# kawshik8/GAN-Image-Captioning

Hardware: AMD Instinct MI355X
Metric: captions/sec (G+D train step) (higher is better)
Workload: dtype bf16; 1 GPU; cfg2: adversarial G+D step, batch 64/GPU, 224x224 images, caption len 20, V=10000, E=H=512, 1-layer LSTM G, CNN-seq D (R=64,F=900), ResNet-50-shaped encoder, --conditional-gan 1; global_batch=64, caption_len=20, image_size=224, vocab=10000, conditional_gan=1, encoder=resnet50, step_impl=fused, parallelism=dp1

## Files before the change

gan-image-captioning_amd/csrc/gemm.h:

```cpp
#pragma once
#include "common.h"

namespace gic {

enum GemmEpi { EPI_PLAIN = 0, EPI_HIGHWAY = 1, EPI_BNSTATS = 2, EPI_GUMBELMAX = 3 };

struct GemmDesc {
  const void* A = nullptr;
  const void* B = nullptr;
  void* C = nullptr;
  int M = 0, N = 0, K = 0;
  long lda = 0, ldb = 0, ldc = 0;
  int a_kc = 1, b_kc = 1;
  int in_dtype = DT_F32, out_dtype = DT_F32;
  const float* bias = nullptr;
  int accumulate = 0;
  int c_zeroed = 0;
  int no_split = 0;
  float alpha = 1.f;
  int epi = EPI_PLAIN;
  const void* X = nullptr; long ldx = 0;
  union { float* Hpre = nullptr; float* a_sum2; };
  union { long ldh = 0; long ldc2; };
  const uint8_t* mask = nullptr; long ldmask = 0;
  uint8_t* mask_out = nullptr; long ldmask_out = 0;
  float keep_scale = 1.f;
  union { int use_philox = 0; int wgrad; }; float drop_p = 0.f; uint64_t seed = 0, stream = 0;
  const uint64_t* seed_dev = nullptr;
  int conv = 0;
  int cH = 0, cW = 0, cCin = 0, cHo = 0, cWo = 0, cKH = 0, cKW = 0, cStride = 1, cPad = 0;
  union { float* stats = nullptr; float* a_sum; };
  int stats_nrep = 1;
  const float* in_stats = nullptr; int in_nrep = 1;
  const float* in_gamma = nullptr; const float* in_beta = nullptr;
  float in_inv_count = 0.f;
  const void* res = nullptr;
  const float* res_stats = nullptr; int res_nrep = 1;
  const float* res_gamma = nullptr; const float* res_beta = nullptr;
  float res_inv_count = 0.f;
  union { void* out_wb = nullptr; void* C2; };
  unsigned long long* gm_rowkey = nullptr;
  const float* gm_bias = nullptr;
  const float* gm_u = nullptr; long gm_ldu = 0;
  float gm_temperature = 1.f;
  int n_fast = 0;
  union { int stats_only = 0; int n_split; };
  int dbg = 0;
};

int gemm(const GemmDesc& d, hipStream_t stream);


struct ConvBase {
  const void* A; const void* B; void* C; float* stats;
  const float* in_stats; const float* in_gamma; const float* in_beta;
  int M, N, lda, ldb, ldc, stats_nrep, in_nrep;
  float in_inv_count;
  unsigned a_bytes, b_bytes;
};

inline bool bn_in_args_ok(const GemmDesc& d) { return d.in_gamma && d.in_beta && d.in_inv_count > 0.f; }

bool conv_base(const GemmDesc& d, long a_elems, long b_elems, ConvBase& b);

bool wgrad_folds_a_sum(const GemmDesc& d);
int wgrad_tile_n(const GemmDesc& d);
void wgrad_launch_counts(long* launches, long* two_matrix);

bool route_only();
char* route_line();
constexpr int kRouteLen = 160;

int gemm_gumbelmax(const GemmDesc& d, hipStream_t stream);
long gemm_gumbelmax_from_cols(int in_dtype, int M, int K, long lda, long ldb);

}
```

gan-image-captioning_amd/csrc/gemm.hip:

```cpp
#include "gemm.h"
#include "conv3x3.h"
#include "conv1x1_stream.h"
#include "conv1x1_panel.h"
#include "conv1x1_pix.h"
#include "conv_stem.h"
#include "bn_fold.h"
#include "gemm_device.h"
#include "kernels.h"

#include <stdlib.h>
#include <string.h>
#include <atomic>

namespace gic {

namespace {

typedef __attribute__((address_space(3))) bf16x4 lds_bf16x4;
typedef const __attribute__((address_space(1))) u32x4* gptr_u4;

__device__ __attribute__((aligned(16))) unsigned int g_zero16[4] = {0u, 0u, 0u, 0u};
typedef const __attribute__((address_space(1))) void* gbl_void_ptr;

#ifdef GIC_STAMPS
}
__device__ unsigned long long g_stamp[32];
namespace {
#define STAMP(i) do { if (tid == 0 && blockIdx.y == 0 && (blockIdx.x == 0 || blockIdx.x == gridDim.x - 1)) { \
  const int o_ = blockIdx.x == 0 ? 0 : 16; g_stamp[o_ + 2 * (i)] = __builtin_amdgcn_s_memtime(); g_stamp[o_ + 2 * (i) + 1] = __builtin_amdgcn_s_memrealtime(); } } while (0)
#define DBG d.dbg
#else
#define STAMP(i) do {} while (0)
#define DBG 0
#endif

template <typename T> struct GlobalPtr { typedef const __attribute__((address_space(1))) T* type; };

template <typename TI, bool KC, int BR, int S, int NC>
__device__ __forceinline__ void g4_store(unsigned char* img, const u32x4 (&reg)[NC], const int tid) {
#pragma unroll
  for (int i = 0; i < NC; ++i) {
    const int c = tid + i * 256;
    if constexpr (KC) {
      *(u32x4*)(img + (c >> 3) * S + (c & 7) * 16) = reg[i];
    } else {
      constexpr int CPR = BR / (16 / (int)sizeof(TI));
      *(u32x4*)(img + (c / CPR) * S + (c % CPR) * 16) = reg[i];
    }
  }
}
template <typename TI, bool KC, int BR, int S>
__device__ __forceinline__ void g4_store_scalar(unsigned char* img, const typename GlobalPtr<TI>::type P, const long ld, const int row0,
                                                const int R, const int k0, const int K, const int tid) {
  constexpr int SZ = sizeof(TI), BK = 128 / SZ;
  for (int e = tid; e < BR * BK; e += 256) {
    TI v = (TI)0.f;
    if constexpr (KC) {
      const int row = e / BK, kk = e % BK;
      const int r = row0 + row, k = k0 + kk;
      if (r < R && k < K) v = P[(long)r * ld + k];
      *(TI*)(img + row * S + kk * SZ) = v;
    } else {
      const int kk = e / BR, row = e % BR;
      const int r = row0 + row, k = k0 + kk;
      if (r < R && k < K) v = P[(long)k * ld + r];
      *(TI*)(img + kk * S + row * SZ) = v;
    }
  }
}
template <bool KC, bool PIPE, int S>
__device__ __forceinline__ bf16x8 g4_frag_bf16(const unsigned char* img, const int r0, const int ks, const int lr, const int lg) {
  if constexpr (PIPE) {
    return *(const bf16x8*)(img + (r0 + lr) * 128 + swz_chunk(r0 + lr, ks * 4 + lg));
  } else if constexpr (KC) {
    return *(const bf16x8*)(img + (r0 + lr) * S + ks * 64 + lg * 16);
  } else {
    const unsigned char* p0 = img + (ks * 32 + lg * 8 + (lr >> 2)) * S + (r0 + 4 * (lr & 3)) * 2;
    const bf16x4 t0 = __builtin_amdgcn_ds_read_tr16_b64_v4bf16((lds_bf16x4*)p0);
    const bf16x4 t1 = __builtin_amdgcn_ds_read_tr16_b64_v4bf16((lds_bf16x4*)(p0 + 4 * S));
    return __builtin_shufflevector(t0, t1, 0, 1, 2, 3, 4, 5, 6, 7);
  }
}
template <bool KC, bool PIPE, int S>
__device__ __forceinline__ void g4_frag_f32(float (&f)[8], const unsigned char* img, const int r0, const int lr, const int lg) {
  if constexpr (KC) {
    const int row = r0 + lr;
    const float4 v0 = *(const float4*)(img + row * S + (PIPE ? swz_chunk(row, 2 * lg) : 2 * lg * 16));
    const float4 v1 = *(const float4*)(img + row * S + (PIPE ? swz_chunk(row, 2 * lg + 1) : (2 * lg + 1) * 16));
    f[0] = v0.x; f[1] = v0.y; f[2] = v0.z; f[3] = v0.w;
    f[4] = v1.x; f[5] = v1.y; f[6] = v1.z; f[7] = v1.w;
  } else {
#pragma unroll
    for (int s = 0; s < 8; ++s) f[s] = *(const float*)(img + (lg * 8 + s) * S + (r0 + lr) * 4);
  }
}

std::atomic<long> g_wgrad_launches{0}, g_wgrad_two{0};

constexpr int EPI_WGRAD = 4;

__device__ __forceinline__ void g4_chunk_add(float (&s)[8], const u32x4 r) {
  const bf16x8 v = __builtin_bit_cast(bf16x8, r);
#pragma unroll
  for (int e = 0; e < 8; ++e) s[e] += (float)v[e];
}

template <typename TI, typename TO, bool AKC, bool BKC, int BM, int BN, bool VEC, int EPI, bool CONV, bool PIPE>
__global__ __launch_bounds__(256) void gemm_kernel(const GemmDesc d, const int k_tiles_per_split) {
  static_assert(!CONV || (AKC && BKC && VEC), "the implicit-GEMM convolution loader is k-contiguous and vectorised");
  static_assert(!PIPE || (AKC && BKC && VEC), "the LDS-DMA pipeline needs k-contiguous 16-byte chunks");
  constexpr bool WG = EPI == EPI_WGRAD;
  static_assert(!WG || (!AKC && !BKC && VEC && !CONV && !PIPE && sizeof(TI) == 2), "the weight-gradient extras exist in the vectorised m/n-contiguous bf16 form only");
  constexpr int SZ = sizeof(TI);
  constexpr int BK = 128 / SZ;
  constexpr int VE = 16 / SZ;
  constexpr int SA = PIPE ? 128 : (AKC ? 144 : BM * SZ + 16);
  constexpr int SB = PIPE ? 128 : (BKC ? 144 : BN * SZ + 16);
  constexpr int NSTAGE = PIPE ? 3 : 2;
  constexpr int A_BYTES = AKC ? BM * SA : BK * SA;
  constexpr int B_BYTES = BKC ? BN * SB : BK * SB;
  constexpr int BUF_BYTES = A_BYTES + B_BYTES;
  constexpr int TM = BM / 32, TN = BN / 32;
  constexpr int CA = BM / 32, CB = BN / 32;
  constexpr bool IS_BF16 = (SZ == 2);
  typedef typename GlobalPtr<TI>::type gptr_t;

  constexpr int EPI_BYTES = BM * (BN * (int)sizeof(TO) + 16) + 4 * (BN / 2) * 2 * 4;
  constexpr int SMEM_BYTES = NSTAGE * BUF_BYTES > EPI_BYTES ? NSTAGE * BUF_BYTES : EPI_BYTES;
  __shared__ __attribute__((aligned(16))) unsigned char smem[SMEM_BYTES];

  const int tid = threadIdx.x, lane = tid & 63, w = tid >> 6;
  STAMP(0);
  const int wr = w >> 1, wc = w & 1;
  const int lr = lane & 15, lg = lane >> 4;

  const int tiles_m = (d.M + BM - 1) / BM;
  const int bid = xcd_run(blockIdx.x, gridDim.x);
  const int bm0 = (bid % tiles_m) * BM;
  const int bn0 = (bid / tiles_m) * BN;

  gptr_t A = (gptr_t)d.A;
  gptr_t B = (gptr_t)d.B;
  const int M = d.M, N = d.N, K = d.K;
  const long lda = d.lda, ldb = d.ldb;

  f32x4 acc[TM][TN];
#pragma unroll
  for (int i = 0; i < TM; ++i)
#pragma unroll
    for (int j = 0; j < TN; ++j) acc[i][j] = (f32x4){0.f, 0.f, 0.f, 0.f};

  u32x4 ra[CA], rb[CB];

  float asum[WG ? VE : 1];
  bool asum_on = false;
  if constexpr (WG) {
    asum_on = d.a_sum && bn0 == 0;
#pragma unroll
    for (int e = 0; e < VE; ++e) asum[e] = 0.f;
  }

  long cv_base[CONV ? CA : 1];
  int cv_hi0[CONV ? CA : 1], cv_wi0[CONV ? CA : 1];
  int cv_r = 0, cv_s = 0, cv_c = 0;
  if constexpr (CONV) {
#pragma unroll
    for (int i = 0; i < CA; ++i) {
      const int m = bm0 + ((tid + i * 256) >> 3);
      const ConvOrigin<long> o = conv_origin<long>(m, m < M, d.cHo, d.cWo, d.cH, d.cW, d.cStride, d.cPad);
      cv_hi0[i] = o.hi0; cv_wi0[i] = o.wi0; cv_base[i] = o.pix;
    }
    const int kchunk = PIPE ? swz_dma_chunk(tid) : (tid & 7);
    const int k = blockIdx.y * k_tiles_per_split * BK + kchunk * VE;
    cv_c = k % d.cCin;
    const int t = k / d.cCin;
    cv_s = t % d.cKW;
    cv_r = t / d.cKW;
  }

  auto gload = [&](int kt) {
    if constexpr (VEC) {
      const int k0 = kt * BK;
      if constexpr (CONV) {
#pragma unroll
        for (int i = 0; i < CA; ++i) {
          ra[i] = (u32x4){0u, 0u, 0u, 0u};
          const int hi = cv_hi0[i] + cv_r, wi = cv_wi0[i] + cv_s;
          if (cv_r < d.cKH && hi >= 0 && hi < d.cH && wi >= 0 && wi < d.cW)
            ra[i] = *(gptr_u4)(A + (cv_base[i] + (long)cv_r * d.cW + cv_s) * d.cCin + cv_c);
        }
      } else {
#pragma unroll
        for (int i = 0; i < CA; ++i) {
          const int c = tid + i * 256;
          ra[i] = (u32x4){0u, 0u, 0u, 0u};
          if constexpr (AKC) {
            const int m = bm0 + (c >> 3), k = k0 + (c & 7) * VE;
            if (m < M && k < K) ra[i] = *(gptr_u4)(A + (long)m * lda + k);
          } else {
            constexpr int CPR = BM / VE;
            const int k = k0 + c / CPR, m = bm0 + (c % CPR) * VE;
            if (k < K && m < M) ra[i] = *(gptr_u4)(A + (long)k * lda + m);
          }
        }
      }
#pragma unroll
      for (int i = 0; i < CB; ++i) {
        const int c = tid + i * 256;
        rb[i] = (u32x4){0u, 0u, 0u, 0u};
        if constexpr (BKC) {
          const int n = bn0 + (c >> 3), k = k0 + (c & 7) * VE;
          if (n < N && k < K) rb[i] = *(gptr_u4)(B + (long)n * ldb + k);
        } else {
          constexpr int CPR = BN / VE;
          const int k = k0 + c / CPR, n = bn0 + (c % CPR) * VE;
          if (k < K && n < N) rb[i] = *(gptr_u4)(B + (long)k * ldb + n);
        }
      }
      if constexpr (CONV) conv_tap_advance(cv_r, cv_s, cv_c, BK, d.cCin, d.cKW);
    }
  };

  auto sstore = [&](int kt, int buf) {
    unsigned char* sA = smem + buf * BUF_BYTES;
    unsigned char* sB = sA + A_BYTES;
    if constexpr (VEC) {
      if constexpr (WG) {
        if (asum_on) {
#pragma unroll
          for (int i = 0; i < CA; ++i) g4_chunk_add(asum, ra[i]);
        }
      }
      g4_store<TI, AKC, BM, SA>(sA, ra, tid);
      g4_store<TI, BKC, BN, SB>(sB, rb, tid);
    } else {
      g4_store_scalar<TI, AKC, BM, SA>(sA, A, lda, bm0, M, kt * BK, K, tid);
      g4_store_scalar<TI, BKC, BN, SB>(sB, B, ldb, bn0, N, kt * BK, K, tid);
    }
  };

  auto issue = [&](int kt, int buf) {
    if constexpr (PIPE) {
      unsigned char* sA = smem + buf * BUF_BYTES;
      unsigned char* sB = sA + A_BYTES;
      const int k0 = kt * BK;
      const int kc = swz_dma_chunk(tid) * VE;
      const int wbase = (tid & ~63) * 16;
#pragma unroll
      for (int i = 0; i < CA; ++i) {
        const int c = tid + i * 256;
        const TI* src = (const TI*)g_zero16;
        if constexpr (CONV) {
          const int hi = cv_hi0[i] + cv_r, wi = cv_wi0[i] + cv_s;
          if (cv_r < d.cKH && hi >= 0 && hi < d.cH && wi >= 0 && wi < d.cW)
            src = (const TI*)d.A + (cv_base[i] + (long)cv_r * d.cW + cv_s) * d.cCin + cv_c;
        } else {
          const int m = bm0 + (c >> 3), k = k0 + kc;
          if (m < M && k < K) src = (const TI*)d.A + (long)m * lda + k;
        }
        __builtin_amdgcn_global_load_lds((gbl_void_ptr)src, (lds_void_ptr)(sA + i * 4096 + wbase), 16, 0, 0);
      }
#pragma unroll
      for (int i = 0; i < CB; ++i) {
        const int c = tid + i * 256;
        const TI* src = (const TI*)g_zero16;
        const int n = bn0 + (c >> 3), k = k0 + kc;
        if (n < N && k < K) src = (const TI*)d.B + (long)n * ldb + k;
        __builtin_amdgcn_global_load_lds((gbl_void_ptr)src, (lds_void_ptr)(sB + i * 4096 + wbase), 16, 0, 0);
      }
      if constexpr (CONV) conv_tap_advance(cv_r, cv_s, cv_c, BK, d.cCin, d.cKW);
    }
  };

  auto compute = [&](int buf) {
    const unsigned char* sA = smem + buf * BUF_BYTES;
    const unsigned char* sB = sA + A_BYTES;
    if constexpr (IS_BF16) {
#pragma unroll
      for (int ks = 0; ks < BK / 32; ++ks) {
        bf16x8 fa[TM], fb[TN];
#pragma unroll
        for (int t = 0; t < TM; ++t) fa[t] = g4_frag_bf16<AKC, PIPE, SA>(sA, wr * (BM / 2) + t * 16, ks, lr, lg);
#pragma unroll
        for (int t = 0; t < TN; ++t) fb[t] = g4_frag_bf16<BKC, PIPE, SB>(sB, wc * (BN / 2) + t * 16, ks, lr, lg);
        mfma_block(acc, fa, fb);
      }
    } else {
      float fa[TM][8], fb[TN][8];
#pragma unroll
      for (int t = 0; t < TM; ++t) g4_frag_f32<AKC, PIPE, SA>(fa[t], sA, wr * (BM / 2) + t * 16, lr, lg);
#pragma unroll
      for (int t = 0; t < TN; ++t) g4_frag_f32<BKC, PIPE, SB>(fb[t], sB, wc * (BN / 2) + t * 16, lr, lg);
#pragma unroll
      for (int s = 0; s < 8; ++s)
#pragma unroll
        for (int i = 0; i < TM; ++i)
#pragma unroll
          for (int j = 0; j < TN; ++j)
            acc[i][j] = __builtin_amdgcn_mfma_f32_16x16x4f32(fa[i][s], fb[j][s], acc[i][j], 0, 0, 0);
    }
  };

  const int nk = (K + BK - 1) / BK;
  const int kt0 = blockIdx.y * k_tiles_per_split;
  const int kt1 = min(nk, kt0 + k_tiles_per_split);
  if constexpr (PIPE) {
    if (kt0 < kt1) {
      constexpr int NL = CA + CB;
      STAMP(1);
      issue(kt0, 0);
      if (kt0 + 1 < kt1) issue(kt0 + 1, 1);
      int buf = 0;
      for (int kt = kt0; kt < kt1; ++kt) {
        if (kt + 1 < kt1) asm volatile("s_waitcnt vmcnt(%0)" ::"n"(NL) : "memory");
        else asm volatile("s_waitcnt vmcnt(0)" ::: "memory");
        __builtin_amdgcn_s_barrier();
        if (kt == kt0) STAMP(2);
        if (kt + 2 < kt1 && !(DBG & 1)) issue(kt + 2, buf >= 1 ? buf - 1 : 2);
        if (!(DBG & 2)) compute(buf);
        buf = buf == 2 ? 0 : buf + 1;
      }
      __syncthreads();
      STAMP(3);
    }
  } else if (kt0 < kt1) {
    int cur = 0;
    gload(kt0);
    sstore(kt0, 0);
    __syncthreads();
    for (int kt = kt0; kt < kt1; ++kt) {
      const bool more = kt + 1 < kt1;
      if (more) gload(kt + 1);
      compute(cur);
      if (more) sstore(kt + 1, cur ^ 1);
      __syncthreads();
      cur ^= 1;
    }
  }

  TO* __restrict__ C = (TO*)d.C;
  long ldc = d.ldc;
#define LDC (WG ? ldc : d.ldc)
  const bool split = gridDim.y > 1;

  if constexpr (WG) {
    if (d.C2 && bn0 >= d.n_split) { C = (TO*)d.C2 - d.n_split; ldc = d.ldc2; }
    if (asum_on) {
      constexpr int CPR = BM / VE, G = 256 / CPR;
      static_assert(G * BM * 4 <= SMEM_BYTES, "the column-sum partials must fit the LDS allocation");
      float* sS = (float*)smem;
#pragma unroll
      for (int e = 0; e < VE; ++e) sS[(tid / CPR) * BM + (tid % CPR) * VE + e] = asum[e];
      __syncthreads();
      if (tid < BM && bm0 + tid < M) {
        float t = 0.f;
#pragma unroll
        for (int g = 0; g < G; ++g) t += sS[g * BM + tid];
        const int m = bm0 + tid;
        if (split) {
          atomicAdd(d.a_sum + m, t);
          if (d.a_sum2) atomicAdd(d.a_sum2 + m, t);
        } else {
          d.a_sum[m] = d.accumulate ? d.a_sum[m] + t : t;
          if (d.a_sum2) d.a_sum2[m] = d.accumulate ? d.a_sum2[m] + t : t;
        }
      }
      __syncthreads();
    }
  }

  if constexpr (EPI != EPI_HIGHWAY) {
    constexpr int OSZ = sizeof(TO);
    constexpr int OVE = 16 / OSZ;
    constexpr int SC = BN * OSZ + 16;
    static_assert(BM * SC + 4 * (BN / 2) * 2 * 4 <= SMEM_BYTES, "C tile + stats scratch must fit the LDS allocation");
    const bool staged = !split && !d.accumulate && (N % OVE == 0) && (LDC % OVE == 0) && ((((uintptr_t)(WG ? (const void*)C : (const void*)d.C)) & 15) == 0);
    if (staged) {
      unsigned char* sC = smem;
      float* sStat = (float*)(smem + BM * SC);
      float st_s[TN], st_q[TN];
#pragma unroll
      for (int j = 0; j < TN; ++j) {
        const int nl = wc * (BN / 2) + j * 16 + lr;
        const int n = bn0 + nl;
        const float bias = (d.bias && n < N) ? d.bias[n] : 0.f;
        st_s[j] = 0.f; st_q[j] = 0.f;
#pragma unroll
        for (int i = 0; i < TM; ++i) {
#pragma unroll
          for (int r = 0; r < 4; ++r) {
            const int ml = wr * (BM / 2) + i * 16 + lg * 4 + r;
            const float v = d.alpha * acc[i][j][r] + bias;
            *(TO*)(sC + ml * SC + nl * OSZ) = from_f32<TO>(v);
            if (EPI == EPI_BNSTATS && bm0 + ml < M) { st_s[j] += v; st_q[j] += v * v; }
          }
        }
        if constexpr (EPI == EPI_BNSTATS) {
          st_s[j] += __shfl_xor(st_s[j], 16, 64); st_q[j] += __shfl_xor(st_q[j], 16, 64);
          st_s[j] += __shfl_xor(st_s[j], 32, 64); st_q[j] += __shfl_xor(st_q[j], 32, 64);
          if (lg == 0) { sStat[(w * (BN / 2) + j * 16 + lr) * 2] = st_s[j]; sStat[(w * (BN / 2) + j * 16 + lr) * 2 + 1] = st_q[j]; }
        }
      }
      __syncthreads();
      STAMP(4);
      if constexpr (EPI == EPI_BNSTATS) {
        if (tid < BN) {
          const int cwc = tid / (BN / 2), cl = tid % (BN / 2), n = bn0 + tid;
          if (n < N) {
            const float s0 = sStat[((0 * 2 + cwc) * (BN / 2) + cl) * 2] + sStat[((1 * 2 + cwc) * (BN / 2) + cl) * 2];
            const float q0 = sStat[((0 * 2 + cwc) * (BN / 2) + cl) * 2 + 1] + sStat[((1 * 2 + cwc) * (BN / 2) + cl) * 2 + 1];
            float* st = d.stats + (long)(blockIdx.x % d.stats_nrep) * 2 * N;
            atomicAdd(&st[n], s0);
            atomicAdd(&st[N + n], q0);
          }
        }
      }
      constexpr int CPR = BN / OVE;
      for (int c = tid; c < BM * CPR; c += 256) {
        const int ml = c / CPR, cc = c % CPR;
        const int m = bm0 + ml, n = bn0 + cc * OVE;
        if (m < M && n < N) *(u32x4*)(C + (long)m * LDC + n) = *(const u32x4*)(sC + ml * SC + cc * 16);
      }
      STAMP(5);
      return;
    }
  }

#pragma unroll
  for (int i = 0; i < TM; ++i) {
#pragma unroll
    for (int j = 0; j < TN; ++j) {
      const int n = bn0 + wc * (BN / 2) + j * 16 + lr;
      if (n >= N) continue;
      const float bias = (d.bias && blockIdx.y == 0) ? d.bias[n] : 0.f;
      const int mb = bm0 + wr * (BM / 2) + i * 16 + lg * 4;
      float keep4[4] = {1.f, 1.f, 1.f, 1.f};
      if constexpr (EPI == EPI_HIGHWAY) {
        if (!d.mask && d.use_philox) highway_keep4(d.seed_dev ? *d.seed_dev : d.seed, d.stream, mb >> 2, N, n, d.drop_p, keep4);
      }
      float st_s = 0.f, st_q = 0.f;
#pragma unroll
      for (int r = 0; r < 4; ++r) {
        const int m = mb + r;
        if (m >= M) continue;
        float v = d.alpha * acc[i][j][r] + bias;
        if constexpr (EPI == EPI_BNSTATS) {
          C[(long)m * LDC + n] = from_f32<TO>(v);
          st_s += v; st_q += v * v;
        } else if constexpr (EPI == EPI_PLAIN || WG) {
          const long o = (long)m * LDC + n;
          if constexpr (sizeof(TO) == 4) {
            if (split) { atomicAdd((float*)&C[o], v); continue; }
          }
          if (d.accumulate) v += to_f32<TO>(C[o]);
          C[o] = from_f32<TO>(v);
        } else {
          const float y = highway_gate(v, to_f32<TI>(((const TI*)d.X)[(long)m * d.ldx + n]));
          if (d.Hpre) d.Hpre[(long)m * d.ldh + n] = v;
          float keep = keep4[r];
          if (d.mask) keep = (float)d.mask[(long)m * d.ldmask + n];
          if (d.mask_out) d.mask_out[(long)m * d.ldmask_out + n] = (uint8_t)keep;
          C[(long)m * LDC + n] = from_f32<TO>(y * keep * d.keep_scale);
        }
      }
      if constexpr (EPI == EPI_BNSTATS) {
        st_s += __shfl_xor(st_s, 16, 64); st_q += __shfl_xor(st_q, 16, 64);
        st_s += __shfl_xor(st_s, 32, 64); st_q += __shfl_xor(st_q, 32, 64);
        float* st = d.stats + (long)(blockIdx.x % d.stats_nrep) * 2 * N;
        if (lg == 0) { atomicAdd(&st[n], st_s); atomicAdd(&st[N + n], st_q); }
      }
    }
  }
}
#undef LDC

template <typename TO, int BN, int EPI, bool CONV, int NS, bool ABN = false, bool ARES = false, int AMAXK = (ARES ? 2048 : 1024)>
__global__ __launch_bounds__(512) void tile8_kernel(const GemmDesc d, const unsigned a_bytes, const unsigned b_bytes) {
  static_assert(!ARES || ABN, "the residual-on-load form extends the A-side BatchNorm");
  constexpr int BM = 128, BK = 64, NT = 512;
  constexpr int TM = 2, TN = BN / 32;
  constexpr int CA = BM * 8 / NT, CB = BN * 8 / NT;
  constexpr int NL = CA + CB + (ARES ? CA : 0);
  constexpr int A_BYTES = BM * 128, B_BYTES = BN * 128, R_BYTES = ARES ? A_BYTES : 0, STAGE = A_BYTES + B_BYTES + R_BYTES;
  constexpr int OSZ = sizeof(TO), OVE = 16 / OSZ, SC = BN * OSZ + 16;
  constexpr int EPI_BYTES = EPI == EPI_HIGHWAY ? BM * (BN + 4) * 4 : (EPI == EPI_GUMBELMAX ? 8 * BN * 4 : BM * SC + 8 * (BN / 2) * 2 * 4);
  constexpr int RING_BYTES = NS * STAGE > EPI_BYTES ? NS * STAGE : EPI_BYTES;
  constexpr int ABN_MAXK = AMAXK;
  constexpr int SMEM_BYTES = RING_BYTES + (ABN ? ABN_MAXK * 8 : 0) + (ARES ? ABN_MAXK * 8 : 0);
  constexpr unsigned OOB = 0x80000000u;
  static_assert(CB >= 1 && SMEM_BYTES <= 160 * 1024, "tile8 LDS budget");
  __shared__ __attribute__((aligned(16))) unsigned char smem[SMEM_BYTES];

  const int tid = threadIdx.x, lane = tid & 63, w = tid >> 6;
  STAMP(0);
  const int wr = w >> 1, wc = w & 1;
  const int lr = lane & 15, lg = lane >> 4;

  const int tiles_m = (d.M + BM - 1) / BM, tiles_n = (d.N + BN - 1) / BN;
  const int bid = xcd_run(blockIdx.x, gridDim.x);
  const int bm0 = (d.n_fast ? bid / tiles_n : bid % tiles_m) * BM;
  const int bn0 = (d.n_fast ? bid % tiles_n : bid / tiles_m) * BN;
  const int M = d.M, N = d.N, K = d.K;

  const __amdgpu_buffer_rsrc_t rsA = __builtin_amdgcn_make_buffer_rsrc((void*)d.A, 0, (int)a_bytes, 0x00020000);
  const __amdgpu_buffer_rsrc_t rsB = __builtin_amdgcn_make_buffer_rsrc((void*)d.B, 0, (int)b_bytes, 0x00020000);
  const __amdgpu_buffer_rsrc_t rsR = __builtin_amdgcn_make_buffer_rsrc((void*)(ARES ? d.res : d.A), 0, (int)a_bytes, 0x00020000);

  const int kc = swz_dma_chunk(tid) * 8;
  int a_off[CA], a_hi0[CA], a_wi0[CA];
  bool a_ok[CA];
  int cv_r = 0, cv_s = 0, cv_c = 0;
#pragma unroll
  for (int i = 0; i < CA; ++i) {
    const int m = bm0 + (tid >> 3) + i * 64;
    a_ok[i] = m < M;
    if constexpr (CONV) {
      const ConvOrigin<int> o = conv_origin<int>(m, a_ok[i], d.cHo, d.cWo, d.cH, d.cW, d.cStride, d.cPad);
      a_hi0[i] = o.hi0; a_wi0[i] = o.wi0;
      a_off[i] = o.pix * d.cCin;
    } else {
      a_hi0[i] = a_wi0[i] = 0;
      a_off[i] = m * (int)d.lda;
    }
  }
  if constexpr (CONV) {
    cv_c = kc % d.cCin;
    const int t = kc / d.cCin;
    cv_s = t % d.cKW;
    cv_r = t / d.cKW;
  }
  int b_off[CB];
  bool b_ok[CB];
#pragma unroll
  for (int i = 0; i < CB; ++i) {
    const int n = bn0 + (tid >> 3) + i * 64;
    b_ok[i] = n < N;
    b_off[i] = n * (int)d.ldb;
  }
  const int wbase = (tid & ~63) * 16;

  auto issue = [&](int kt, int st) {
    unsigned char* sA = smem + st * STAGE;
    unsigned char* sB = sA + A_BYTES;
    const int k = kt * BK + kc;
    const bool kok = k < K;
#pragma unroll
    for (int i = 0; i < CA; ++i) {
      unsigned voff;
      if constexpr (CONV) {
        const bool ok = (unsigned)(a_hi0[i] + cv_r) < (unsigned)d.cH & (unsigned)(a_wi0[i] + cv_s) < (unsigned)d.cW & kok;
        voff = ok ? (unsigned)(a_off[i] + (cv_r * d.cW + cv_s) * d.cCin + cv_c) * 2u : OOB;
      } else {
        voff = (a_ok[i] & kok) ? (unsigned)(a_off[i] + k) * 2u : OOB;
      }
      __builtin_amdgcn_raw_ptr_buffer_load_lds(rsA, (lds_void_ptr)(sA + i * (NT * 16) + wbase), 16, (int)voff, 0, 0, CONV ? GIC_TRUNK_NT : 0);
      if constexpr (ARES)
        __builtin_amdgcn_raw_ptr_buffer_load_lds(rsR, (lds_void_ptr)(sB + B_BYTES + i * (NT * 16) + wbase), 16, (int)voff, 0, 0, CONV ? GIC_TRUNK_NT : 0);
    }
#pragma unroll
    for (int i = 0; i < CB; ++i) {
      const unsigned voff = (b_ok[i] & kok) ? (unsigned)(b_off[i] + k) * 2u : OOB;
      __builtin_amdgcn_raw_ptr_buffer_load_lds(rsB, (lds_void_ptr)(sB + i * (NT * 16) + wbase), 16, (int)voff, 0, 0, 0);
    }
    if constexpr (CONV) conv_tap_advance(cv_r, cv_s, cv_c, BK, d.cCin, d.cKW);
  };

  float* coef = (float*)(smem + RING_BYTES);
  if constexpr (ABN) {
    const int Cn = CONV ? d.cCin : K;
    for (int c = tid; c < ABN_MAXK; c += NT) {
      float sc = 0.f, sh = 0.f;
      if (c < Cn) {
        float mean, rstd;
        bn_moments(d.in_stats, d.in_nrep, Cn, c, d.in_inv_count, mean, rstd);
        sc = d.in_gamma[c] * rstd;
        sh = d.in_beta[c] - mean * sc;
      }
      coef[2 * c] = sc; coef[2 * c + 1] = sh;
      if constexpr (ARES) {
        float rs = 1.f, rt = 0.f;
        if (d.res_stats && c < Cn) {
          float mean, rstd;
          bn_moments(d.res_stats, d.res_nrep, Cn, c, d.res_inv_count, mean, rstd);
          rs = d.res_gamma[c] * rstd;
          rt = d.res_beta[c] - mean * rs;
        }
        coef[2 * ABN_MAXK + 2 * c] = rs; coef[2 * ABN_MAXK + 2 * c + 1] = rt;
      }
    }
    __syncthreads();
  }
  const bool wb = ARES && d.out_wb && bn0 == 0;
  auto abn = [&](int kt, int st) {
    if constexpr (ABN) {
      const int k = kt * BK + kc;
      if (k < K) {
        const int ch = CONV ? k % d.cCin : k;
        const int tap = CONV ? k / d.cCin : 0;
        const int ts = tap % (CONV ? d.cKW : 1), tr = tap / (CONV ? d.cKW : 1);
        float scl[8], sft[8];
        bn_unpack8(coef + 2 * ch, scl, sft);
        float rsc[8] = {1.f, 1.f, 1.f, 1.f, 1.f, 1.f, 1.f, 1.f}, rsf[8] = {0.f, 0.f, 0.f, 0.f, 0.f, 0.f, 0.f, 0.f};
        if constexpr (ARES) bn_unpack8(coef + 2 * ABN_MAXK + 2 * ch, rsc, rsf);
#pragma unroll
        for (int i = 0; i < CA; ++i) {
          const bool ok = CONV ? ((unsigned)(a_hi0[i] + tr) < (unsigned)d.cH & (unsigned)(a_wi0[i] + ts) < (unsigned)d.cW) : a_ok[i];
          if (!ok) continue;
          bf16x8* p = (bf16x8*)(smem + st * STAGE + i * (NT * 16) + tid * 16);
          bf16x8 v = *p;
          if constexpr (ARES) {
            const bf16x8 r = *(const bf16x8*)(smem + st * STAGE + A_BYTES + B_BYTES + i * (NT * 16) + tid * 16);
#pragma unroll
            for (int e = 0; e < 8; ++e) v[e] = (bf16_t)fmaxf((float)v[e] * scl[e] + sft[e] + ((float)r[e] * rsc[e] + rsf[e]), 0.f);
            if (wb) *(bf16x8*)((bf16_t*)d.out_wb + (long)a_off[i] + k) = v;
          } else {
            v = bn_relu8(v, scl, sft);
          }
          *p = v;
        }
      }
    }
  };

  f32x4 acc[TM][TN];
#pragma unroll
  for (int i = 0; i < TM; ++i)
#pragma unroll
    for (int j = 0; j < TN; ++j) acc[i][j] = (f32x4){0.f, 0.f, 0.f, 0.f};

  auto compute = [&](int st) {
    const unsigned char* sA = smem + st * STAGE;
    const unsigned char* sB = sA + A_BYTES;
    bf16x8 fa[2][TM], fb[2][TN];
#pragma unroll
    for (int ks = 0; ks < 2; ++ks) {
#pragma unroll
      for (int t = 0; t < TM; ++t) {
        const int row = wr * 32 + t * 16 + lr;
        fa[ks][t] = *(const bf16x8*)(sA + row * 128 + swz_chunk(row, ks * 4 + lg));
      }
// ... 360 lines not shown
  p.vec = vec;
  const bool bf16_in = d.in_dtype == DT_BF16;
  p.tiles = cdiv(d.M, p.bm) * cdiv(d.N, p.bm);
  const int tiles = p.tiles, nk = cdiv(d.K, bf16_in ? 64 : 32);
  int splits = 1;
  if (d.epi == EPI_PLAIN && bf16_in && d.out_dtype == DT_F32 && !d.no_split) {
    if (tiles < 24 && nk >= 8) {
      splits = 256 / tiles;
      if (splits > nk / 2) splits = nk / 2;
      if (splits > 16) splits = 16;
    } else if (tiles <= 192 && nk >= 32) {
      splits = 512 / tiles;
      if (splits > nk / 8) splits = nk / 8;
      if (splits > 16) splits = 16;
    } else if (!d.a_kc && !d.b_kc && tiles <= 192 && nk >= 16) {
      splits = 512 / tiles;
      if (splits > nk / 4) splits = nk / 4;
    } else if (tiles <= 320 && nk >= 64) {
      splits = 768 / tiles;
    }
    if (splits < 1) splits = 1;
    if (det_mode()) splits = (d.accumulate || splits < 2) ? 1 : 2;
  }
  p.per = nk ? cdiv(nk, splits) : 1;
  p.splits = nk ? cdiv(nk, p.per) : 1;
  p.zero_grid = 0;
  if (p.splits > 1 && !d.accumulate && !d.c_zeroed) {
    const long total = (long)d.M * d.N;
    p.zero_grid = (int)((total + 255) / 256 > 1024 ? 1024 : (total + 255) / 256);
  }
  static const bool no_pipe = getenv("GIC_GEMM_NO_PIPE") != nullptr;
  p.pipe = d.a_kc && d.b_kc && vec && p.per >= 6 && (long)tiles * p.splits <= 2 * 256 + 8 && !no_pipe;
  p.wg = wgrad_form(d, vec) && (d.a_sum || d.C2);
}

int select(const GemmDesc& d, bool vec, int after, Plan& p) {
  const bool bf16_in = d.in_dtype == DT_BF16, bf16_out = d.out_dtype == DT_BF16;
  if (!((d.in_dtype == DT_F32 && d.out_dtype == DT_F32) || (bf16_in && (d.out_dtype == DT_F32 || bf16_out)))) {
    set_last_error("gemm: unsupported dtypes in=%d out=%d", d.in_dtype, d.out_dtype);
    return GIC_ERR_UNSUPPORTED;
  }
  if (d.conv) {
    if (!vec || !d.a_kc || !d.b_kc) { set_last_error("gemm: convolution needs 16-B aligned NHWC / KRSC operands"); return GIC_ERR_UNSUPPORTED; }
    if (bf16_in != bf16_out || (d.epi != EPI_BNSTATS && d.epi != EPI_PLAIN)) {
      set_last_error("gemm: unsupported convolution epilogue / dtype");
      return GIC_ERR_UNSUPPORTED;
    }
  } else if (d.epi != EPI_PLAIN && d.epi != EPI_HIGHWAY) {
    set_last_error("gemm: unknown epilogue %d", d.epi);
    return GIC_ERR_UNSUPPORTED;
  }
  auto take = [&](int family) { p.family = family; return GIC_OK; };
  if (d.conv && bf16_out && d.epi == EPI_BNSTATS) {
    if (after < F_STEM && select_conv_stem(d, p.stem)) return take(F_STEM);
    if (after < F_PATCH && select_conv3x3_patch(d, p.patch)) return take(F_PATCH);
    if (after < F_STREAM && select_conv1x1_stream(d, p.strm)) return take(F_STREAM);
    if (d.stats_only) return GIC_ERR_UNSUPPORTED;
    if (after < F_PIX && select_conv1x1_pix(d, p.pix)) return take(F_PIX);
    if (after < F_PANEL && select_conv1x1_panel(d, p.panel)) return take(F_PANEL);
    if (d.in_stats && d.cKH * d.cKW > 1) return GIC_ERR_UNSUPPORTED;
  }
  if (after < F_TILE8 && bf16_in && (d.conv || (d.a_kc && d.b_kc && vec))) {
    p.d = d;
    if (select_tile8(d, p.t8, p.d.n_fast)) return take(F_TILE8);
  }
  if (d.conv && d.in_stats) return GIC_ERR_UNSUPPORTED;
  if (!(d.a_kc && d.b_kc) && (d.epi != EPI_PLAIN || d.b_kc)) {
    set_last_error("gemm: unsupported layout a_kc=%d b_kc=%d epi=%d", d.a_kc, d.b_kc, d.epi);
    return GIC_ERR_UNSUPPORTED;
  }
  p.d = d;
  select_gemm4(d, vec, p.g4);
  if (!d.conv && d.epi == EPI_PLAIN && d.C2 && !(p.g4.wg && d.n_split > 0 && d.n_split < d.N && d.n_split % p.g4.bm == 0)) {
    set_last_error("gemm: a second output needs the vectorised weight-gradient form and n_split (%d) on a tile boundary (%d)", d.n_split, p.g4.bm);
    return GIC_ERR_UNSUPPORTED;
  }
  return take(F_GEMM4);
}

long gumbelmax_from_cols(int in_dtype, int M, int K, long lda, long ldb) {
  static const bool off = getenv("GIC_NO_TILE8") != nullptr || getenv("GIC_NO_FUSED_GUMBELMAX") != nullptr;
  if (off || in_dtype != DT_BF16 || M < 128 || M % 4 || K % 8 || lda % 8 || ldb % 8 || !under_2g(kc_extent(M, lda, K))) return 0;
  const long mt = cdiv(M, 128), nt = (160 + mt - 1) / mt;
  return 128 * (nt - 1) + 1 > 128 ? 128 * (nt - 1) + 1 : 128;
}

bool select_gumbelmax(const GemmDesc& d0, Plan& p) {
  GemmDesc& d = p.d = d0;
  const long from = gumbelmax_from_cols(d.in_dtype, d.M, d.K, d.lda, d.ldb);
  if (!from || d.N < from || !d.a_kc || !d.b_kc || !aligned16(d.A) || !aligned16(d.B) || !aligned16(d.gm_bias) ||
      (d.gm_u && (!aligned16(d.gm_u) || d.gm_ldu % 4)) || !(d.gm_temperature > 0.f))
    return false;
  const long a_elems = kc_extent(d.M, d.lda, d.K), b_elems = kc_extent(d.N, d.ldb, d.K);
  const long tiles = (long)cdiv(d.M, 128) * cdiv(d.N, 128);
  if (!under_2g(b_elems)) return false;
  d.epi = EPI_GUMBELMAX;
  d.n_fast = xcd_share_a(2l * d.M * d.K, 2l * d.N * d.K, cdiv(d.N, 128));
  p.t8 = {128, tiles > 256 ? 2 : 4, false, false, 1024, (unsigned)tiles, (unsigned)(a_elems * 2), (unsigned)(b_elems * 2)};
  p.family = F_TILE8;
  return true;
}


__global__ void zero2d_kernel(float* __restrict__ C, long ldc, int M, int N) {
  const long total = (long)M * N;
  for (long i = (long)blockIdx.x * blockDim.x + threadIdx.x; i < total; i += (long)gridDim.x * blockDim.x)
    C[(i / N) * ldc + (i % N)] = 0.f;
}

__global__ void zero_wgrad_kernel(float* __restrict__ C, long ldc, float* __restrict__ C2, long ldc2, int n_split, float* __restrict__ s1,
                                  float* __restrict__ s2, int M, int N) {
  const long total = (long)M * N, i0 = (long)blockIdx.x * blockDim.x + threadIdx.x, step = (long)gridDim.x * blockDim.x;
  for (long i = i0; i < total; i += step) {
    const long m = i / N;
    const int n = (int)(i - m * N);
    if (C2 && n >= n_split) C2[m * ldc2 + (n - n_split)] = 0.f;
    else C[m * ldc + n] = 0.f;
  }
  for (long m = i0; m < M; m += step) {
    if (s1) s1[m] = 0.f;
    if (s2) s2[m] = 0.f;
  }
}

template <typename TO, int EPI, bool CONV, int BN, int NS, bool ABN = false, bool ARES = false, int AMAXK = 1024>
void launch_tile8_as(const Plan& p, hipStream_t stream) {
  if constexpr (!ABN || (EPI == EPI_BNSTATS && CONV))
    if (EPI != EPI_HIGHWAY || NS != 1)
      hipLaunchKernelGGL((tile8_kernel<TO, BN, EPI, CONV, NS, ABN, ARES, AMAXK>), dim3(p.t8.grid), dim3(512), 0, stream, p.d, p.t8.a_bytes, p.t8.b_bytes);
}

constexpr int t8_key(int BN, int NS, bool abn = false, bool ares = false, int amaxk = 1024) { return BN + NS * 256 + abn * 2048 + ares * 4096 + amaxk * 8192; }

template <typename TO, int EPI, bool CONV>
void launch_tile8_variant(const Plan& p, hipStream_t stream) {
  const Tile8Plan& t = p.t8;
  switch (t8_key(t.BN, t.NS, t.abn, t.ares, t.amaxk)) {
#define GIC_T8(...) case t8_key(__VA_ARGS__): return launch_tile8_as<TO, EPI, CONV, __VA_ARGS__>(p, stream)
    GIC_T8(128, 1); GIC_T8(128, 2); GIC_T8(128, 4); GIC_T8(64, 1); GIC_T8(64, 2); GIC_T8(64, 4);
    GIC_T8(128, 1, true); GIC_T8(128, 2, true); GIC_T8(128, 4, true); GIC_T8(64, 1, true); GIC_T8(64, 2, true); GIC_T8(64, 4, true);
    GIC_T8(128, 1, true, true, 512); GIC_T8(128, 2, true, true, 512); GIC_T8(64, 1, true, true, 512); GIC_T8(64, 2, true, true, 512);
    GIC_T8(128, 1, true, true, 2048); GIC_T8(128, 2, true, true, 2048); GIC_T8(64, 1, true, true, 2048); GIC_T8(64, 2, true, true, 2048);
#undef GIC_T8
  }
}

void launch_tile8(const Plan& p, hipStream_t stream) {
  const GemmDesc& d = p.d;
  const bool bf16_out = d.out_dtype == DT_BF16;
  if (d.epi == EPI_GUMBELMAX) {
    if (p.t8.NS == 2) launch_tile8_as<float, EPI_GUMBELMAX, false, 128, 2>(p, stream);
    else launch_tile8_as<float, EPI_GUMBELMAX, false, 128, 4>(p, stream);
  } else if (d.conv) {
    if (d.epi == EPI_BNSTATS) launch_tile8_variant<bf16_t, EPI_BNSTATS, true>(p, stream);
    else launch_tile8_variant<bf16_t, EPI_PLAIN, true>(p, stream);
  } else if (d.epi == EPI_HIGHWAY) {
    launch_tile8_variant<bf16_t, EPI_HIGHWAY, false>(p, stream);
  } else {
    if (bf16_out) launch_tile8_variant<bf16_t, EPI_PLAIN, false>(p, stream);
    else launch_tile8_variant<float, EPI_PLAIN, false>(p, stream);
  }
}

template <typename TI, typename TO, bool AKC, bool BKC, int BM, bool VEC, int EPI, bool CONV>
void launch_gemm4_as(const Plan& p, hipStream_t stream) {
  const dim3 grid(p.g4.tiles, p.g4.splits);
  if constexpr (AKC && BKC && VEC) {
    if (p.g4.pipe) {
      hipLaunchKernelGGL((gemm_kernel<TI, TO, AKC, BKC, BM, BM, VEC, EPI, CONV, true>), grid, dim3(256), 0, stream, p.d, p.g4.per);
      return;
    }
  }
  hipLaunchKernelGGL((gemm_kernel<TI, TO, AKC, BKC, BM, BM, VEC, EPI, CONV, false>), grid, dim3(256), 0, stream, p.d, p.g4.per);
}

template <typename TI, typename TO, bool AKC, bool BKC, int EPI, bool CONV>
void launch_gemm4_tile(const Plan& p, hipStream_t stream) {
  const bool big = p.g4.bm == 128;
  if (CONV || p.g4.vec) return big ? launch_gemm4_as<TI, TO, AKC, BKC, 128, true, EPI, CONV>(p, stream) : launch_gemm4_as<TI, TO, AKC, BKC, 64, true, EPI, CONV>(p, stream);
  if constexpr (!CONV && EPI != EPI_WGRAD) return big ? launch_gemm4_as<TI, TO, AKC, BKC, 128, false, EPI, CONV>(p, stream) : launch_gemm4_as<TI, TO, AKC, BKC, 64, false, EPI, CONV>(p, stream);
}

template <typename TI, typename TO>
void launch_gemm4_typed(const Plan& p, hipStream_t stream) {
  const GemmDesc& d = p.d;
  if (d.conv) {
    if constexpr (sizeof(TI) == sizeof(TO)) {
      if (d.epi == EPI_BNSTATS) launch_gemm4_tile<TI, TO, true, true, EPI_BNSTATS, true>(p, stream);
      else launch_gemm4_tile<TI, TO, true, true, EPI_PLAIN, true>(p, stream);
    }
  } else if (d.epi == EPI_HIGHWAY) {
    launch_gemm4_tile<TI, TO, true, true, EPI_HIGHWAY, false>(p, stream);
  } else if (d.a_kc) {
    if (d.b_kc) launch_gemm4_tile<TI, TO, true, true, EPI_PLAIN, false>(p, stream);
    else launch_gemm4_tile<TI, TO, true, false, EPI_PLAIN, false>(p, stream);
  } else if (p.g4.wg) {
    if constexpr (sizeof(TI) == 2) launch_gemm4_tile<TI, TO, false, false, EPI_WGRAD, false>(p, stream);
  } else {
    launch_gemm4_tile<TI, TO, false, false, EPI_PLAIN, false>(p, stream);
  }
}

void launch_gemm4(const Plan& p, hipStream_t stream) {
  const GemmDesc& d = p.d;
  if (p.g4.wg) {
    g_wgrad_launches.fetch_add(1, std::memory_order_relaxed);
    if (d.C2) g_wgrad_two.fetch_add(1, std::memory_order_relaxed);
  }
  if (p.g4.zero_grid && p.g4.wg)
    hipLaunchKernelGGL(zero_wgrad_kernel, dim3(p.g4.zero_grid), dim3(256), 0, stream, (float*)d.C, d.ldc, (float*)d.C2, d.ldc2, d.n_split, d.a_sum, d.a_sum2, d.M, d.N);
  else if (p.g4.zero_grid) hipLaunchKernelGGL(zero2d_kernel, dim3(p.g4.zero_grid), dim3(256), 0, stream, (float*)d.C, d.ldc, d.M, d.N);
  if (d.in_dtype == DT_F32) launch_gemm4_typed<float, float>(p, stream);
  else if (d.out_dtype == DT_F32) launch_gemm4_typed<bf16_t, float>(p, stream);
  else launch_gemm4_typed<bf16_t, bf16_t>(p, stream);
}

bool launch(const Plan& p, hipStream_t stream) {
  switch (p.family) {
    case F_STEM: return launch_conv_stem(p.stem, stream);
    case F_PATCH: return launch_conv3x3_patch(p.patch, stream);
    case F_STREAM: return launch_conv1x1_stream(p.strm, stream);
    case F_PIX: return launch_conv1x1_pix(p.pix, stream);
    case F_PANEL: return launch_conv1x1_panel(p.panel, stream);
    case F_TILE8: launch_tile8(p, stream); return true;
    default: launch_gemm4(p, stream); return true;
  }
}

const char* const kFamily[] = {"none", "conv stem", "conv3x3 patch", "conv1x1 stream", "conv1x1 pix", "conv1x1 panel", "gemm tile8", "gemm"};

void write_route(const Plan& p) {
  char* s = route_line();
  const GemmDesc& d = p.d;
  const char* tn[] = {"f32", "bf16"};
  auto b = [](bool v) { return v ? "true" : "false"; };
  switch (p.family) {
    case F_STEM: snprintf(s, kRouteLen, "conv_stem grid=%u block=512 lds=%zu", p.stem.grid, p.stem.lds); break;
    case F_PATCH: snprintf(s, kRouteLen, "conv3x3_patch<%d,%d,%s,%s> grid=%u block=512 lds=%zu", p.patch.BN, p.patch.P, b(p.patch.multi), b(p.patch.abn), p.patch.grid, p.patch.lds); break;
    case F_STREAM: snprintf(s, kRouteLen, "conv1x1_stream<%d,%d,%s,%s> grid=%u block=512 lds=%zu", p.strm.BN, p.strm.KT, b(p.strm.abn), b(p.strm.stats), p.strm.grid, p.strm.lds); break;
    case F_PIX: snprintf(s, kRouteLen, "conv1x1_pix<%d,%d,%s> grid=%u block=512 lds=%zu", p.pix.K, p.pix.NSTG, b(p.pix.turn), p.pix.grid, p.pix.lds); break;
    case F_PANEL: snprintf(s, kRouteLen, "conv1x1_panel<%d,%s> grid=%u block=512 lds=%zu", p.panel.KT, b(p.panel.abn), p.panel.grid, p.panel.lds); break;
    case F_TILE8:
      snprintf(s, kRouteLen, "tile8<%s,%d,%d,%s,%d,%s,%s,%d> grid=%u block=512 lds=0", d.epi == EPI_GUMBELMAX ? "f32" : tn[d.out_dtype], p.t8.BN, d.epi, b(d.conv),
               p.t8.NS, b(p.t8.abn), b(p.t8.ares), p.t8.amaxk, p.t8.grid);
      break;
    default:
      snprintf(s, kRouteLen, "gemm<%s,%s,%s,%s,%d,%d,%s,%d,%s,%s> grid=%dx%d block=256 lds=0 splits=%d per=%d pipe=%d zero=%d", tn[d.in_dtype], tn[d.out_dtype],
               b(d.a_kc), b(d.b_kc), p.g4.bm, p.g4.bm, b(d.conv || p.g4.vec), d.epi, b(d.conv), b(p.g4.pipe), p.g4.tiles, p.g4.splits, p.g4.splits, p.g4.per,
               (int)p.g4.pipe, p.g4.zero_grid);
      if (p.g4.wg) {
        const size_t n = strlen(s);
        snprintf(s + n, kRouteLen - n, " a_sum=%d n_split=%d", d.a_sum ? (d.a_sum2 ? 2 : 1) : 0, d.C2 ? d.n_split : 0);
      }
  }
}

}

bool conv_base(const GemmDesc& d, long a_elems, long b_elems, ConvBase& b) {
  if (!d.conv || d.epi != EPI_BNSTATS || !d.stats || d.in_dtype != DT_BF16 || d.out_dtype != DT_BF16) return false;
  if (d.bias || d.alpha != 1.f || d.accumulate || !aligned16(d.A) || !aligned16(d.B) || !aligned16(d.C)) return false;
  if (d.in_stats && (!bn_in_args_ok(d) || d.in_nrep < 1)) return false;
  if (a_elems * 2 >= (1l << 31) || b_elems * 2 >= (1l << 31)) return false;
  b.A = d.A; b.B = d.B; b.C = d.C; b.stats = d.stats;
  b.in_stats = d.in_stats; b.in_gamma = d.in_gamma; b.in_beta = d.in_beta;
  b.M = d.M; b.N = d.N; b.lda = (int)d.lda; b.ldb = (int)d.ldb; b.ldc = (int)d.ldc;
  b.stats_nrep = d.stats_nrep < 1 ? 1 : d.stats_nrep; b.in_nrep = d.in_nrep; b.in_inv_count = d.in_inv_count;
  b.a_bytes = (unsigned)(a_elems * 2); b.b_bytes = (unsigned)(b_elems * 2);
  return true;
}

void wgrad_launch_counts(long* launches, long* two_matrix) {
  if (launches) *launches = g_wgrad_launches.load(std::memory_order_relaxed);
  if (two_matrix) *two_matrix = g_wgrad_two.load(std::memory_order_relaxed);
}

bool wgrad_folds_a_sum(const GemmDesc& d) { return d.a_sum && wgrad_form(d, plain_vec(d)); }

int wgrad_tile_n(const GemmDesc& d) {
  const bool vec = plain_vec(d);
  if (!wgrad_form(d, vec)) return 0;
  Gemm4Plan p;
  select_gemm4(d, vec, p);
  return p.bm;
}

long gemm_gumbelmax_from_cols(int in_dtype, int M, int K, long lda, long ldb) { return gumbelmax_from_cols(in_dtype, M, K, lda, ldb); }

int gemm_gumbelmax(const GemmDesc& d, hipStream_t stream) {
  GIC_CHECK_ARG(d.A && d.B && d.gm_rowkey && d.gm_bias, "gemm_gumbelmax: null operand");
  Plan p;
  const bool ok = select_gumbelmax(d, p), probe = route_only();
  if (probe && ok) write_route(p);
  if (probe && !ok) snprintf(route_line(), kRouteLen, "unsupported");
  if (!ok) return GIC_ERR_UNSUPPORTED;
  if (probe) return GIC_OK;
  launch_tile8(p, stream);
  GIC_CHECK_LAUNCH("gemm gumbelmax");
  return GIC_OK;
}

int gemm(const GemmDesc& d0, hipStream_t stream) {
  GemmDesc d = d0;
#ifdef GIC_STAMPS
  { const char* e = getenv("GIC_GEMM_DBG"); if (e) d.dbg = atoi(e); }
#endif
  static const bool log = getenv("GIC_GEMM_LOG") != nullptr;
  const bool probe = route_only();
  if (probe) route_line()[0] = 0;
  GIC_CHECK_ARG(d.A && d.B && d.C, "gemm: null operand");
  GIC_CHECK_ARG(d.M >= 0 && d.N >= 0 && d.K >= 0, "gemm: negative dim");
  if (d.M == 0 || d.N == 0) return GIC_OK;
  if (d.epi == EPI_HIGHWAY) GIC_CHECK_ARG(d.X, "gemm: highway epilogue needs X");
  const int sz = dtype_size(d.in_dtype);
  const int ve = 16 / sz;
  bool vec = plain_vec(d);
  if (d.conv) {
    const bool chunk_ok = (d.cCin % ve == 0) || (d.cPad == 0 && ve % d.cCin == 0 && (d.cKW * d.cCin) % ve == 0);
    GIC_CHECK_ARG(chunk_ok && d.K == d.cKH * d.cKW * d.cCin && d.K % ve == 0, "gemm: conv needs Cin %% %d == 0 (or a pre-padded NHWC4 stem) and K = KH*KW*Cin", ve);
    GIC_CHECK_ARG(d.epi != EPI_BNSTATS || d.stats, "gemm: EPI_BNSTATS needs a stats buffer");
    vec = aligned16(d.A) && aligned16(d.B) && (d.ldb % ve == 0);
  }
  Plan p;
  for (int after = F_NONE;; after = p.family) {
    const int rc = select(d, vec, after, p);
    if (log || probe) {
      if (rc == GIC_OK) write_route(p);
      else snprintf(route_line(), kRouteLen, "unsupported");
      if (log && !d.conv)
        fprintf(stderr, "[gemm] M=%d N=%d K=%d a_kc=%d b_kc=%d in=%d out=%d epi=%d acc=%d -> %s\n", d.M, d.N, d.K, d.a_kc, d.b_kc, d.in_dtype, d.out_dtype,
                d.epi, d.accumulate, route_line());
    }
    if (rc != GIC_OK || probe) return rc;
    if (launch(p, stream)) break;
  }
  GIC_CHECK_LAUNCH(kFamily[p.family]);
  return GIC_OK;
}

}
#ifdef GIC_STAMPS
extern "C" int gic_debug_stamps(unsigned long long* out) {
  return (int)hipMemcpyFromSymbol(out, HIP_SYMBOL(gic::g_stamp), sizeof(unsigned long long) * 32);
}
#endif
```

Before: 26650 captions/s.

## Add two-deep register-staged prefetch to the 64x64 bf16 GEMM main loop

For the non-pipelined, vectorised bf16 64x64 GEMM tiles, the kernel now keeps NSET (default 2) register sets of global-load chunks in flight. A new branchless zero-page chunk loader feeds them, so more memory latency is hidden behind the MFMA compute of the current LDS buffer. It also adds an amdgpu_waves_per_eu hint of 4 for that variant to cap register use. The costs are extra VGPRs, padded zero iterations when the K-tile count is not a multiple of NSET, and a getenv call on every gemm invocation, now done outside the stamps build.

```diff
diff --git a/gan-image-captioning_amd/csrc/gemm.h b/gan-image-captioning_amd/csrc/gemm.h
--- a/gan-image-captioning_amd/csrc/gemm.h
+++ b/gan-image-captioning_amd/csrc/gemm.h
@@ -4,6 +4,8 @@
 namespace gic {
 
 enum GemmEpi { EPI_PLAIN = 0, EPI_HIGHWAY = 1, EPI_BNSTATS = 2, EPI_GUMBELMAX = 3 };
+
+constexpr int GEMM_DBG_ONE_TILE = 256;
 
 struct GemmDesc {
   const void* A = nullptr;
diff --git a/gan-image-captioning_amd/csrc/gemm.hip b/gan-image-captioning_amd/csrc/gemm.hip
--- a/gan-image-captioning_amd/csrc/gemm.hip
+++ b/gan-image-captioning_amd/csrc/gemm.hip
@@ -95,9 +95,32 @@
   }
 }
 
+template <typename TI, bool KC, int BR>
+__device__ __forceinline__ u32x4 g4_chunk_load(const typename GlobalPtr<TI>::type P, const long ld, const int row0, const int R, const int k0,
+                                               const int K, const int c, const bool live) {
+  constexpr int VE = 16 / (int)sizeof(TI);
+  int r, k;
+  if constexpr (KC) {
+    r = row0 + (c >> 3); k = k0 + (c & 7) * VE;
+  } else {
+    constexpr int CPR = BR / VE;
+    k = k0 + c / CPR; r = row0 + (c % CPR) * VE;
+  }
+  gptr_u4 p = (gptr_u4)g_zero16;
+  if (live && r < R && k < K) p = (gptr_u4)(P + (KC ? (long)r * ld + k : (long)k * ld + r));
+  return *p;
+}
+
 std::atomic<long> g_wgrad_launches{0}, g_wgrad_two{0};
 
 constexpr int EPI_WGRAD = 4;
+
+template <typename TI, int BM, int BN, bool VEC, bool CONV, bool PIPE>
+constexpr bool g4_deep = !PIPE && VEC && !CONV && sizeof(TI) == 2 && BM == 64 && BN == 64;
+
+#ifndef GIC_GEMM_STAGE_SETS
+#define GIC_GEMM_STAGE_SETS 2
+#endif
 
 __device__ __forceinline__ void g4_chunk_add(float (&s)[8], const u32x4 r) {
   const bf16x8 v = __builtin_bit_cast(bf16x8, r);
@@ -106,7 +129,7 @@
 }
 
 template <typename TI, typename TO, bool AKC, bool BKC, int BM, int BN, bool VEC, int EPI, bool CONV, bool PIPE>
-__global__ __launch_bounds__(256) void gemm_kernel(const GemmDesc d, const int k_tiles_per_split) {
+__global__ __launch_bounds__(256) __attribute__((amdgpu_waves_per_eu(g4_deep<TI, BM, BN, VEC, CONV, PIPE> ? 4 : 1))) void gemm_kernel(const GemmDesc d, const int k_tiles_per_split) {
   static_assert(!CONV || (AKC && BKC && VEC), "the implicit-GEMM convolution loader is k-contiguous and vectorised");
   static_assert(!PIPE || (AKC && BKC && VEC), "the LDS-DMA pipeline needs k-contiguous 16-byte chunks");
   constexpr bool WG = EPI == EPI_WGRAD;
@@ -150,7 +173,10 @@
 #pragma unroll
     for (int j = 0; j < TN; ++j) acc[i][j] = (f32x4){0.f, 0.f, 0.f, 0.f};
 
+  constexpr bool DEEP = g4_deep<TI, BM, BN, VEC, CONV, PIPE>;
+  constexpr int NSET = DEEP ? GIC_GEMM_STAGE_SETS : 1;
   u32x4 ra[CA], rb[CB];
+  u32x4 xa[DEEP ? NSET - 1 : 1][CA], xb[DEEP ? NSET - 1 : 1][CB];
 
   float asum[WG ? VE : 1];
   bool asum_on = false;
@@ -178,8 +204,13 @@
     cv_r = t / d.cKW;
   }
 
-  auto gload = [&](int kt) {
-    if constexpr (VEC) {
+  auto gload_to = [&](int kt, bool live, u32x4 (&ra)[CA], u32x4 (&rb)[CB]) {
+    if constexpr (DEEP) {
+#pragma unroll
+      for (int i = 0; i < CA; ++i) ra[i] = g4_chunk_load<TI, AKC, BM>(A, lda, bm0, M, kt * BK, K, tid + i * 256, live);
+#pragma unroll
+      for (int i = 0; i < CB; ++i) rb[i] = g4_chunk_load<TI, BKC, BN>(B, ldb, bn0, N, kt * BK, K, tid + i * 256, live);
+    } else if constexpr (VEC) {
       const int k0 = kt * BK;
       if constexpr (CONV) {
 #pragma unroll
@@ -221,7 +252,7 @@
     }
   };
 
-  auto sstore = [&](int kt, int buf) {
+  auto sstore_from = [&](int kt, int buf, const u32x4 (&ra)[CA], const u32x4 (&rb)[CB]) {
     unsigned char* sA = smem + buf * BUF_BYTES;
     unsigned char* sB = sA + A_BYTES;
     if constexpr (VEC) {
@@ -238,6 +269,9 @@
       g4_store_scalar<TI, BKC, BN, SB>(sB, B, ldb, bn0, N, kt * BK, K, tid);
     }
   };
+
+  auto gload = [&](int kt) { gload_to(kt, true, ra, rb); };
+  auto sstore = [&](int kt, int buf) { sstore_from(kt, buf, ra, rb); };
 
   auto issue = [&](int kt, int buf) {
     if constexpr (PIPE) {
@@ -324,18 +358,45 @@
       STAMP(3);
     }
   } else if (kt0 < kt1) {
+    bool one_tile = true;
+    if constexpr (DEEP) one_tile = (d.dbg & GEMM_DBG_ONE_TILE) != 0 || kt1 - kt0 <= NSET;
     int cur = 0;
-    gload(kt0);
-    sstore(kt0, 0);
-    __syncthreads();
-    for (int kt = kt0; kt < kt1; ++kt) {
-      const bool more = kt + 1 < kt1;
-      if (more) gload(kt + 1);
-      compute(cur);
-      if (more) sstore(kt + 1, cur ^ 1);
+    STAMP(1);
+    if (one_tile) {
+      gload(kt0);
+      sstore(kt0, 0);
       __syncthreads();
-      cur ^= 1;
-    }
+      STAMP(2);
+      for (int kt = kt0; kt < kt1; ++kt) {
+        const bool more = kt + 1 < kt1;
+        if (more && !(DBG & 1)) gload(kt + 1);
+        if (!(DBG & 2)) compute(cur);
+        if (more) sstore(kt + 1, cur ^ 1);
+        __syncthreads();
+        cur ^= 1;
+      }
+    } else if constexpr (DEEP) {
+#define SET_A(s) ((s) == 0 ? ra : xa[(s) == 0 ? 0 : (s) - 1])
+#define SET_B(s) ((s) == 0 ? rb : xb[(s) == 0 ? 0 : (s) - 1])
+#pragma unroll
+      for (int s = 0; s < NSET; ++s) gload_to(kt0 + s, kt0 + s < kt1, SET_A(s), SET_B(s));
+      sstore(kt0, 0);
+      __syncthreads();
+      STAMP(2);
+      for (int kt = kt0; kt < kt1; kt += NSET) {
+#pragma unroll
+        for (int s = 0; s < NSET; ++s) {
+          gload_to(kt + s + NSET, kt + s + NSET < kt1 && !(DBG & 1), SET_A(s), SET_B(s));
+          if (!(DBG & 2)) compute(cur);
+          sstore_from(kt + s + 1, cur ^ 1, SET_A((s + 1) % NSET), SET_B((s + 1) % NSET));
+          __syncthreads();
+          cur ^= 1;
+        }
+      }
+#undef SET_A
+#undef SET_B
+    }
+    STAMP(3);
   }
 
   TO* __restrict__ C = (TO*)d.C;
@@ -1302,9 +1363,7 @@
 
 int gemm(const GemmDesc& d0, hipStream_t stream) {
   GemmDesc d = d0;
-#ifdef GIC_STAMPS
   { const char* e = getenv("GIC_GEMM_DBG"); if (e) d.dbg = atoi(e); }
-#endif
   static const bool log = getenv("GIC_GEMM_LOG") != nullptr;
   const bool probe = route_only();
   if (probe) route_line()[0] = 0;
```

Result: no change. 26680 captions/s, median of 5 (+0.1%).
